# google-research/rigl

Measured on AMD Instinct MI355X. Metric: images/sec/node, ResNet-50 80% ERK RigL step, higher is better.
Workload: dtype bf16

## Files before the change

### include/rigl_hip.h

```cpp
#ifndef RIGL_HIP_H_
#define RIGL_HIP_H_

#include <stddef.h>
#include <stdint.h>

#ifdef __cplusplus
extern "C" {
#endif

#define RIGL_ABI_VERSION 2

typedef void* rigl_stream_t;
typedef uint16_t rigl_bf16;

enum {
  RIGL_OK = 0,
  RIGL_EINVAL = -1,
  RIGL_ELAUNCH = -2,
  RIGL_EWORKSPACE = -3,
  RIGL_EUNSUPPORTED = -4
};

int rigl_version(void);
uint32_t rigl_crc32c(const void* data, size_t n, uint32_t crc);
// ... 282 lines not shown
                      const float* gamma, const float* save_mean,
                      const float* save_invstd, const float* save_scale,
                      const float* save_shift, int32_t relu, rigl_bf16* dx,
                      rigl_bf16* dresidual , float* dgamma,
                      float* dbeta, const float* stats, int32_t stats_parts,
                      void* workspace, size_t workspace_bytes, rigl_stream_t stream);

int rigl_bn_add_bn_fwd(int64_t m, int32_t c, const rigl_bf16* x, const rigl_bf16* x2,
                       const float* scale2, const float* shift2,
                       const float* gamma, const float* beta, float* running_mean,
                       float* running_var, float momentum, float eps, int32_t relu,
                       rigl_bf16* y, float* save_mean, float* save_invstd,
                       float* save_scale, float* save_shift, const float* stats,
                       int32_t stats_parts, uint8_t* relu_bits ,
                       void* workspace, size_t workspace_bytes, rigl_stream_t stream);
size_t rigl_bn_add_bn_bwd_workspace_bytes(int64_t m, int32_t c);
int rigl_bn_add_bn_bwd(int64_t m, int32_t c, const rigl_bf16* x, const rigl_bf16* x2,
                       const uint8_t* relu_bits, const rigl_bf16* dy,
                       const float* gamma, const float* save_mean, const float* save_invstd,
                       const float* gamma2, const float* save_mean2, const float* save_invstd2,
                       rigl_bf16* dx, rigl_bf16* dx2, float* dgamma, float* dbeta,
                       float* dgamma2, float* dbeta2, void* workspace,
                       size_t workspace_bytes, rigl_stream_t stream);

int rigl_stateless_random(float* out, int64_t n, int32_t seed0, int32_t seed1,
                          int32_t dist, float scale, float shift,
                          rigl_stream_t stream);
typedef struct {
  float* out;
  int64_t n;
// ... 118 lines not shown
```

### rigl_amd/_lib.py

```python
import ctypes as C
import os

_HERE = os.path.dirname(os.path.abspath(__file__))
ABI_VERSION = 2
LIB_PATH = os.environ.get('RIGL_HIP_LIB') or os.path.join(_HERE, 'lib', 'librigl_hip.so')

RIGL_OK = 0
RIGL_EINVAL = -1
RIGL_ELAUNCH = -2
RIGL_EWORKSPACE = -3
RIGL_EUNSUPPORTED = -4
COUNTS_PER_LAYER = 8
MAGPRUNE_COUNTS_PER_LAYER = 4
PROF_KINDS = ('conv_fwd', 'conv_dgrad', 'conv_wgrad', 'prune_regrow',
              'sgd_momentum', 'pack_weights', 'conv_bwd', 'depthwise', 'masked_adam', 'magnitude_prune')

GROW_ZEROS, GROW_GRAD_SCALE, GROW_GRAD_SIGN, GROW_EXPLICIT = 0, 1, 2, 3
MOMRESET_ZEROS, MOMRESET_GRAD = 0, 1


class RiglError(RuntimeError):

  def __init__(self, code, msg):
    super().__init__('librigl_hip: error %d: %s' % (code, msg))
# ... 124 lines not shown
    'rigl_bn_fwd': (C.c_int, [_I64, _I32, _P, _P, _P, _P, _P, _P, _F, _F, _I32, _P, _P, _P, _P, _P, _P, _SZ, _P]),
    'rigl_bn_fwd_stats': (C.c_int, [_I64, _I32, _P, _P, _P, _P, _P, _P, _F, _F, _I32, _P, _P, _P, _P, _P, _P, _I32, _P, _P, _SZ, _P]),
    'rigl_bn_bwd': (C.c_int, [_I64, _I32, _P, _P, _P, _P, _P, _P, _P, _P, _P, _I32, _P, _P, _P, _P, _P, _SZ, _P]),
    'rigl_bn_bwd_stats': (C.c_int, [_I64, _I32, _P, _P, _P, _P, _P, _P, _P, _P, _P, _I32, _P, _P, _P, _P, _P, _I32, _P, _SZ, _P]),
    'rigl_bn_bwd_reduce': (C.c_int, [_I64, _I32, _P, _P, _P, _P, _P, _P, _I32, _P, _P, _P, _P, _SZ, _P]),
    'rigl_crc32c': (C.c_uint32, [_P, _SZ, C.c_uint32]),
    'rigl_stateless_random': (C.c_int, [_P, _I64, _I32, _I32, _I32, _F, _F, _P]),
    'rigl_stateless_random_batched': (C.c_int, [C.POINTER(RandomItem), _I32, _P]),
    'rigl_dropout_fwd': (C.c_int, [_P, _P, _P, _I64, _I32, _F, _I32, _P, _P]),
    'rigl_dropout_bwd': (C.c_int, [_P, _P, _P, _I64, _I32, _F, _P]),
    'rigl_dropout_advance': (C.c_int, [_P, _P]),
    'rigl_maxpool_fwd': (C.c_int, [C.POINTER(ConvDesc), _P, _P, _P, _P]),
    'rigl_maxpool_bwd': (C.c_int, [C.POINTER(ConvDesc), _P, _P, _P, _P]),
    'rigl_bn_fwd_statistics': (C.c_int, [_I64, _I32, _P, _P, _P, _P, _P, _F, _F, _P, _P, _P, _P, _P, _I32, _P, _SZ, _P]),
    'rigl_bn_add_bn_fwd': (C.c_int, [_I64, _I32, _P, _P, _P, _P, _P, _P, _P, _P, _F, _F, _I32, _P, _P, _P, _P, _P, _P, _I32, _P, _P, _SZ, _P]),
    'rigl_bn_add_bn_bwd_workspace_bytes': (_SZ, [_I64, _I32]),
    'rigl_bn_add_bn_bwd': (C.c_int, [_I64, _I32, _P, _P, _P, _P, _P, _P, _P, _P, _P, _P, _P, _P, _P, _P, _P, _P, _P, _SZ, _P]),
    'rigl_bn_relu_maxpool_fwd': (C.c_int, [C.POINTER(ConvDesc), _P, _P, _P, _P, _P, _P]),
    'rigl_bn_relu_maxpool_bwd_workspace_bytes': (_SZ, [C.POINTER(ConvDesc)]),
    'rigl_bn_relu_maxpool_bwd': (C.c_int, [C.POINTER(ConvDesc), _P, _P, _P, _P, _P, _P, _P, _P, _P, _P, _P, _P, _SZ, _P]),
    'rigl_global_avgpool_fwd': (C.c_int, [_I32, _I32, _I32, _P, _P, _P]),
    'rigl_global_avgpool_bwd': (C.c_int, [_I32, _I32, _I32, _P, _P, _P]),
    'rigl_softmax_xent': (C.c_int, [_I32, _I32, _P, _P, _F, _F, _P, _P, _P]),
    'rigl_global_avgpool_bwd_relu': (C.c_int, [_I32, _I32, _I32, _P, _P, _P, _P]),
    'rigl_conv2d_fwd_takes_relu_epilogue': (C.c_int32, [C.POINTER(ConvDesc)]),
    'rigl_conv2d_bwd_takes_relu_epilogue': (C.c_int32, [C.POINTER(ConvDesc)]),
    'rigl_masked_conv2d_fwd_relu': (C.c_int, [C.POINTER(ConvDesc), _P, _P, _P, _P, _SZ, _P]),
    'rigl_masked_conv2d_bwd_relu': (C.c_int, [C.POINTER(ConvDesc), _P, _P, _P, _P, _P, _P, _SZ, _P]),
    'rigl_relu_fwd': (C.c_int, [_I64, _P, _P, _P]),
    'rigl_relu_bwd': (C.c_int, [_I64, _P, _P, _P, _P]),
# ... 50 lines not shown
```

### rigl_amd/csrc/bn.hip

```cpp
#include "common.hpp"

namespace rigl {
namespace kbn {

constexpr int THREADS = 256;
constexpr int MAX_PARTS = 512;

__device__ __forceinline__ float bf_lo(uint32_t w) { return __uint_as_float(w << 16); }
__device__ __forceinline__ float bf_hi(uint32_t w) { return __uint_as_float(w & 0xFFFF0000u); }
__device__ __forceinline__ uint32_t f2bf(float f) {
  uint32_t u = __float_as_uint(f);
  if ((u & 0x7FFFFFFFu) > 0x7F800000u) return (u >> 16) | 0x40u;
  u += 0x7FFFu + ((u >> 16) & 1u);
  return u >> 16;
}
typedef __attribute__((ext_vector_type(2))) __bf16 bf16x2_t;
typedef __attribute__((ext_vector_type(2))) float f32x2_t;
__device__ __forceinline__ uint32_t pack2(float a, float b) {
  const f32x2_t v = {a, b};
  return __builtin_bit_cast(uint32_t, __builtin_convertvector(v, bf16x2_t));
}
__device__ __forceinline__ void unpack8(const uint4& v, float f[8]) {
  f[0] = bf_lo(v.x); f[1] = bf_hi(v.x); f[2] = bf_lo(v.y); f[3] = bf_hi(v.y);
  f[4] = bf_lo(v.z); f[5] = bf_hi(v.z); f[6] = bf_lo(v.w); f[7] = bf_hi(v.w);
// ... 99 lines not shown
      for (int j = 0; j < 16; ++j) own[j] += oth[j];
      if (s > 1) {
#pragma unroll
        for (int j = 0; j < 16; ++j) red[threadIdx.x][j] = own[j];
      }
    }
    if (s > 1) __syncthreads();
  }
  if (ty == 0 && c_ok) {
    float* p = partial + ((int64_t)blockIdx.x * 2) * G.C + cgi * 8;
#pragma unroll
    for (int j = 0; j < 8; ++j) { p[j] = own[j]; p[G.C + j] = own[8 + j]; }
  }
}

template <int CL>
__device__ __forceinline__ void sum_partials(const Geom& G, const float* __restrict__ partial, double& s0, double& s1,
                                             int& c, bool& leader) {
  constexpr int PL = THREADS / CL;
  __shared__ double acc[2][PL][CL + 1];
  const int cl = threadIdx.x % CL, pl = threadIdx.x / CL;
  c = blockIdx.x * CL + cl;
  double a0 = 0.0, a1 = 0.0;
  if (c < G.C) {
#ifndef RIGL_BN_FIN_FLIGHT
#define RIGL_BN_FIN_FLIGHT 16
#endif
    constexpr int FLIGHT = RIGL_BN_FIN_FLIGHT;
    for (int p0 = pl; p0 < G.parts; p0 += PL * FLIGHT) {
      float v0[FLIGHT], v1[FLIGHT];
#pragma unroll
      for (int j = 0; j < FLIGHT; ++j) {
        const int p = p0 + j * PL;
        const int pc = p < G.parts ? p : G.parts - 1;
        const float l0 = partial[((int64_t)pc * 2) * G.C + c], l1 = partial[((int64_t)pc * 2 + 1) * G.C + c];
        v0[j] = p < G.parts ? l0 : 0.f;
        v1[j] = p < G.parts ? l1 : 0.f;
      }
#pragma unroll
      for (int j = 0; j < FLIGHT; ++j) { a0 += (double)v0[j]; a1 += (double)v1[j]; }
    }
  }
  acc[0][pl][cl] = a0; acc[1][pl][cl] = a1;
  __syncthreads();
  leader = pl == 0 && c < G.C;
  s0 = s1 = 0.0;
  if constexpr (CL == 1) {
    __shared__ double acc2[2][16];
    if (threadIdx.x < 16) {
      double t0 = 0.0, t1 = 0.0;
#pragma unroll
      for (int k = 0; k < 16; ++k) { t0 += acc[0][threadIdx.x * 16 + k][0]; t1 += acc[1][threadIdx.x * 16 + k][0]; }
      acc2[0][threadIdx.x] = t0; acc2[1][threadIdx.x] = t1;
    }
    __syncthreads();
    if (leader) {
#pragma unroll
      for (int k = 0; k < 16; ++k) { s0 += acc2[0][k]; s1 += acc2[1][k]; }
    }
  } else if (leader) {
#pragma unroll 8
    for (int k = 0; k < PL; ++k) { s0 += acc[0][k][cl]; s1 += acc[1][k][cl]; }
  }
}

template <int CL>
__global__ __launch_bounds__(THREADS) void k_fwd_finalize(Geom G, const float* __restrict__ partial,
                                                           const uint16_t* __restrict__ x ,
                                                           const float* __restrict__ gamma, const float* __restrict__ beta,
                                                           float* __restrict__ running_mean, float* __restrict__ running_var,
                                                           float momentum, float eps, float* __restrict__ save_mean,
                                                           float* __restrict__ save_invstd, float* __restrict__ scale,
                                                           float* __restrict__ shift) {
  double s0, s1; int c; bool leader;
  sum_partials<CL>(G, partial, s0, s1, c, leader);
  if (!leader) return;
  const double m = (double)G.M;
  double k = 0.0;
  if (x) {
    const float a = __uint_as_float((uint32_t)x[c] << 16), b = __uint_as_float((uint32_t)x[(G.M / 2) * G.C + c] << 16),
                e = __uint_as_float((uint32_t)x[(G.M - 1) * G.C + c] << 16);
    k = (double)pivot3(a, b, e);
  }
  const double dm = s0 / m;
  const double mean = k + dm;
  double var = s1 / m - dm * dm;
  if (var < 0.0) var = 0.0;
  const float invstd = (float)(1.0 / sqrt(var + (double)eps));
  save_mean[c] = (float)mean;
  save_invstd[c] = invstd;
  const float sc = gamma[c] * invstd;
  scale[c] = sc;
  shift[c] = beta[c] - (float)mean * sc;
  if (running_mean) {
    const double unbiased = G.M > 1 ? var * m / (m - 1.0) : var;
    running_mean[c] = (1.f - momentum) * running_mean[c] + momentum * (float)mean;
    running_var[c] = (1.f - momentum) * running_var[c] + momentum * (float)unbiased;
  }
}

template <bool RELU, bool HAS_RES>
__global__ __launch_bounds__(THREADS) void k_fwd_apply(Geom G, const uint16_t* __restrict__ x, const uint16_t* __restrict__ res,
                                                        const float* __restrict__ scale, const float* __restrict__ shift,
                                                        uint16_t* __restrict__ y, uint8_t* __restrict__ mbits) {
  extern __shared__ __attribute__((aligned(16))) float prm[];
  const bool fixed = G.fixed != 0;
  float psc[8], psh[8];
  if (fixed) {
    const int c0 = (int)(((int64_t)blockIdx.x * THREADS + threadIdx.x) % G.cg) * 8;
    ld8f(scale + c0, psc); ld8f(shift + c0, psh);
  } else {
    for (int i = threadIdx.x; i < G.C; i += THREADS) { prm[i] = scale[i]; prm[G.C + i] = shift[i]; }
    __syncthreads();
// ... 16 lines not shown
      if (HAS_RES) v += rv[j];
      o[j] = RELU ? fmaxf(v, 0.f) : v;
    }
    uint4 out;
    out.x = pack2(o[0], o[1]); out.y = pack2(o[2], o[3]); out.z = pack2(o[4], o[5]); out.w = pack2(o[6], o[7]);
    st16(y + i * 8, out, G.nt);
    if (RELU && mbits) {
      uint32_t mb = 0u;
#pragma unroll
      for (int j = 0; j < 8; ++j) mb |= (o[j] > 0.f ? 1u : 0u) << j;
      mbits[i] = (uint8_t)mb;
    }
  }
}

template <int CL>
__global__ __launch_bounds__(THREADS) void k_bwd_finalize(Geom G, const float* __restrict__ partial,
                                                           const float* __restrict__ gamma, const float* __restrict__ invstd,
                                                           float* __restrict__ dgamma, float* __restrict__ dbeta,
                                                           float* __restrict__ coef ) {
  double s0, s1; int c; bool leader;
  sum_partials<CL>(G, partial, s0, s1, c, leader);
  if (!leader) return;
  dbeta[c] = (float)s0;
  dgamma[c] = (float)s1;
  coef[c] = gamma[c] * invstd[c];
  coef[G.C + c] = (float)(s0 / (double)G.M);
  coef[2 * G.C + c] = (float)(s1 / (double)G.M);
}

template <bool RELU, int MSK, bool HAS_DRES>
__global__ __launch_bounds__(THREADS) void k_bwd_apply(Geom G, const uint16_t* __restrict__ x, const uint16_t* __restrict__ y,
                                                        const uint8_t* __restrict__ mbits,
                                                        const uint16_t* __restrict__ dy, const float* __restrict__ mean,
                                                        const float* __restrict__ invstd, const float* __restrict__ scale,
                                                        const float* __restrict__ shift, const float* __restrict__ coef,
                                                        uint16_t* __restrict__ dx, uint16_t* __restrict__ dres) {
  extern __shared__ __attribute__((aligned(16))) float prm[];
  const bool fixed = G.fixed != 0;
  float pm[8], pis[8], pa[8], pb[8], pc[8], psc[8], psh[8];
  if (fixed) {
// ... 157 lines not shown
    if (s > 1) __syncthreads();
  }
  if (ty == 0 && c_ok) {
    float* p = partial + ((int64_t)blockIdx.x * 2) * G.C + cgi * 8;
    float* p2 = partial2 + ((int64_t)blockIdx.x * 2) * G.C + cgi * 8;
#pragma unroll
    for (int j = 0; j < 8; ++j) {
      p[j] = own[j]; p[G.C + j] = own[8 + j];
      p2[j] = own[j]; p2[G.C + j] = own[16 + j];
    }
  }
}

struct FinSet { const float* partial; const float* gamma; const float* invstd; float* dgamma; float* dbeta; float* coef; };

template <int CL>
__global__ __launch_bounds__(THREADS) void k_bwd_finalize_pair(Geom G, FinSet s0, FinSet s1) {
  const FinSet& f = blockIdx.y == 0 ? s0 : s1;
  double a0, a1; int c; bool leader;
  sum_partials<CL>(G, f.partial, a0, a1, c, leader);
  if (!leader) return;
  f.dbeta[c] = (float)a0;
  f.dgamma[c] = (float)a1;
  f.coef[c] = f.gamma[c] * f.invstd[c];
  f.coef[G.C + c] = (float)(a0 / (double)G.M);
  f.coef[2 * G.C + c] = (float)(a1 / (double)G.M);
}

__global__ __launch_bounds__(THREADS) void k_bwd_apply_pair(Geom G, const uint16_t* __restrict__ x, const uint16_t* __restrict__ x2,
                                                             const uint8_t* __restrict__ mbits, const uint16_t* __restrict__ dy,
                                                             const float* __restrict__ mean, const float* __restrict__ invstd,
                                                             const float* __restrict__ mean2, const float* __restrict__ invstd2,
                                                             const float* __restrict__ coef, const float* __restrict__ coef2,
                                                             uint16_t* __restrict__ dx, uint16_t* __restrict__ dx2) {
  extern __shared__ __attribute__((aligned(16))) float prm[];
  const bool fixed = G.fixed != 0;
  float q[10][8];
  if (fixed) {
    const int c0 = (int)(((int64_t)blockIdx.x * THREADS + threadIdx.x) % G.cg) * 8;
// ... 83 lines not shown

static unsigned apply_grid(Geom& g) {
#ifndef RIGL_BN_APPLY_PER_THREAD
#define RIGL_BN_APPLY_PER_THREAD 2
#endif
#ifndef RIGL_BN_APPLY_CAP
#define RIGL_BN_APPLY_CAP 16384
#endif
  int64_t b = (g.M * g.cg + THREADS * RIGL_BN_APPLY_PER_THREAD - 1) / (THREADS * RIGL_BN_APPLY_PER_THREAD);
  if (b > RIGL_BN_APPLY_CAP) b = RIGL_BN_APPLY_CAP;
  if (b < 1) b = 1;
  g.fixed = (RIGL_TUNE("bn_regs", 1) != 0 && (b * THREADS) % g.cg == 0) ? 1 : 0;
  return (unsigned)b;
}

void launch_bwd_finalize(int64_t m, int c, const float* partial, int parts, const float* gamma, const float* invstd,
                         float* dgamma, float* dbeta, float* coef, hipStream_t st) {
  Geom g = make_geom(m, c);
  g.parts = parts;
  if (parts > MAX_PARTS)
    hipLaunchKernelGGL(k_bwd_finalize<4>, dim3((unsigned)((c + 3) / 4)), dim3(THREADS), 0, st, g, partial, gamma, invstd,
                       dgamma, dbeta, coef);
  else
    hipLaunchKernelGGL(k_bwd_finalize<16>, dim3((unsigned)((c + 15) / 16)), dim3(THREADS), 0, st, g, partial, gamma, invstd,
                       dgamma, dbeta, coef);
}

static int fwd_statistics(Geom& g, int32_t c, const rigl_bf16* x, const float* gamma, const float* beta,
                          float* running_mean, float* running_var, float momentum, float eps, float* save_mean,
                          float* save_invstd, float* save_scale, float* save_shift, const float* stats,
                          int32_t stats_parts, void* workspace, size_t workspace_bytes, hipStream_t st) {
  const float* partial = stats;
  if (!stats) {
    const size_t need = rigl_bn_workspace_bytes(g.M, c);
    if (!workspace || workspace_bytes < need) return fail(RIGL_EWORKSPACE, "rigl_bn_fwd: workspace %zu < %zu", workspace_bytes, need);
    float* ws_partial = static_cast<float*>(workspace);
    dim3 rgrid((unsigned)g.parts, (unsigned)((g.cg + g.tpr - 1) / g.tpr));
    hipLaunchKernelGGL((k_reduce<0, false, 0>), rgrid, dim3(THREADS), 0, st, g, x, nullptr, nullptr, nullptr, nullptr, nullptr,
                       nullptr, nullptr, ws_partial);
    partial = ws_partial;
  } else {
    g.parts = stats_parts;
  }
  if (g.parts > 1024 && RIGL_TUNE("bn_fin1", 1) != 0)
    hipLaunchKernelGGL(k_fwd_finalize<1>, dim3((unsigned)c), dim3(THREADS), 0, st, g, partial, stats ? nullptr : reinterpret_cast<const uint16_t*>(x), gamma,
                       beta, running_mean, running_var, momentum, eps, save_mean, save_invstd, save_scale, save_shift);
  else if (g.parts > 256)
    hipLaunchKernelGGL(k_fwd_finalize<4>, dim3((unsigned)((c + 3) / 4)), dim3(THREADS), 0, st, g, partial, stats ? nullptr : reinterpret_cast<const uint16_t*>(x), gamma,
                       beta, running_mean, running_var, momentum, eps, save_mean, save_invstd, save_scale, save_shift);
  else
    hipLaunchKernelGGL(k_fwd_finalize<16>, dim3((unsigned)((c + 15) / 16)), dim3(THREADS), 0, st, g, partial, stats ? nullptr : reinterpret_cast<const uint16_t*>(x), gamma,
                       beta, running_mean, running_var, momentum, eps, save_mean, save_invstd, save_scale, save_shift);
  return RIGL_OK;
}

}
}

extern "C" {

size_t rigl_bn_workspace_bytes(int64_t m, int32_t c) {
  if (m <= 0 || c <= 0) return 0;
  rigl::kbn::Geom g = rigl::kbn::make_geom(m, c);
  return rigl::align_up((size_t)g.parts * 2 * c * 4, 256) + rigl::align_up((size_t)3 * c * 4, 256);
}

int rigl_bn_fwd_stats(int64_t m, int32_t c, const rigl_bf16* x, const rigl_bf16* residual, const float* gamma,
// ... 61 lines not shown
      !save_scale || !save_shift)
    return fail(RIGL_EINVAL, "rigl_bn_add_bn_fwd: bad arguments");
  if (c % 8) return fail(RIGL_EUNSUPPORTED, "rigl_bn_add_bn_fwd: channels %% 8 != 0");
  if (4 * (size_t)c * 4 > 65536) return fail(RIGL_EUNSUPPORTED, "rigl_bn_add_bn_fwd: too many channels for the LDS parameter cache");
  if (stats && stats_parts <= 0) return fail(RIGL_EINVAL, "rigl_bn_add_bn_fwd: stats_parts must be positive");
  hipStream_t st = as_stream(stream);
  Geom g = make_geom(m, c);
  int rc = fwd_statistics(g, c, x, gamma, beta, running_mean, running_var, momentum, eps, save_mean, save_invstd,
                          save_scale, save_shift, stats, stats_parts, workspace, workspace_bytes, st);
  if (rc) return rc;
  dim3 agrid(apply_grid(g));
  const size_t lds = g.fixed ? 0 : (size_t)4 * c * 4;
  if (relu) hipLaunchKernelGGL(k_fwd_apply_pair<true>, agrid, dim3(THREADS), lds, st, g, x, x2, save_scale, save_shift, scale2, shift2, y, relu_bits);
  else hipLaunchKernelGGL(k_fwd_apply_pair<false>, agrid, dim3(THREADS), lds, st, g, x, x2, save_scale, save_shift, scale2, shift2, y, nullptr);
  RIGL_CHECK_LAUNCH("rigl_bn_add_bn_fwd");
  return RIGL_OK;
}

size_t rigl_bn_add_bn_bwd_workspace_bytes(int64_t m, int32_t c) { return 2 * rigl_bn_workspace_bytes(m, c); }

int rigl_bn_add_bn_bwd(int64_t m, int32_t c, const rigl_bf16* x, const rigl_bf16* x2, const uint8_t* relu_bits,
                       const rigl_bf16* dy, const float* gamma, const float* save_mean, const float* save_invstd,
                       const float* gamma2, const float* save_mean2, const float* save_invstd2, rigl_bf16* dx,
                       rigl_bf16* dx2, float* dgamma, float* dbeta, float* dgamma2, float* dbeta2, void* workspace,
                       size_t workspace_bytes, rigl_stream_t stream) {
  using namespace rigl;
  using namespace rigl::kbn;
  if (m <= 0 || c <= 0 || !x || !x2 || !relu_bits || !dy || !gamma || !save_mean || !save_invstd || !gamma2 || !save_mean2 ||
      !save_invstd2 || !dx || !dx2 || !dgamma || !dbeta || !dgamma2 || !dbeta2)
    return fail(RIGL_EINVAL, "rigl_bn_add_bn_bwd: bad arguments");
// ... 7 lines not shown
  if (lds > 65536 && !big_lds) return fail(RIGL_ELAUNCH, "rigl_bn_add_bn_bwd: cannot raise the dynamic LDS limit");
  hipStream_t st = as_stream(stream);
  Geom g = make_geom(m, c);
  const size_t half = rigl_bn_workspace_bytes(m, c);
  const size_t part_bytes = align_up((size_t)g.parts * 2 * c * 4, 256);
  char* w0 = static_cast<char*>(workspace);
  float* partial = reinterpret_cast<float*>(w0);
  float* coef = reinterpret_cast<float*>(w0 + part_bytes);
  float* partial2 = reinterpret_cast<float*>(w0 + half);
  float* coef2 = reinterpret_cast<float*>(w0 + half + part_bytes);
  dim3 rgrid((unsigned)g.parts, (unsigned)((g.cg + g.tpr - 1) / g.tpr));
  hipLaunchKernelGGL(k_reduce_pair, rgrid, dim3(THREADS), 0, st, g, x, x2, relu_bits, dy, save_mean, save_invstd, save_mean2,
                     save_invstd2, partial, partial2);
  const FinSet f0 = {partial, gamma, save_invstd, dgamma, dbeta, coef};
  const FinSet f1 = {partial2, gamma2, save_invstd2, dgamma2, dbeta2, coef2};
  hipLaunchKernelGGL(k_bwd_finalize_pair<16>, dim3((unsigned)((c + 15) / 16), 2), dim3(THREADS), 0, st, g, f0, f1);
  const dim3 pgrid(apply_grid(g));
  hipLaunchKernelGGL(k_bwd_apply_pair, pgrid, dim3(THREADS), g.fixed ? 0 : lds, st, g, x, x2, relu_bits, dy, save_mean, save_invstd,
                     save_mean2, save_invstd2, coef, coef2, dx, dx2);
  RIGL_CHECK_LAUNCH("rigl_bn_add_bn_bwd");
  return RIGL_OK;
}

static int bn_bwd_impl(int64_t m, int32_t c, const rigl_bf16* x, const rigl_bf16* y, const uint8_t* relu_bits,
                       const rigl_bf16* dy, const float* gamma,
                       const float* save_mean, const float* save_invstd, const float* save_scale, const float* save_shift,
                       int32_t relu, rigl_bf16* dx, rigl_bf16* dresidual, float* dgamma, float* dbeta,
                       const float* stats, int32_t stats_parts, float* coef_out, void* workspace,
                       size_t workspace_bytes, rigl_stream_t stream) {
  using namespace rigl;
  using namespace rigl::kbn;
// ... 12 lines not shown
  float* coef = coef_out ? coef_out : reinterpret_cast<float*>(static_cast<char*>(workspace) + align_up((size_t)g.parts * 2 * c * 4, 256));
  dim3 rgrid((unsigned)g.parts, (unsigned)((g.cg + g.tpr - 1) / g.tpr));
  const int msk = relu_bits ? 2 : (y ? 1 : 0);
  const float* red = partial;
  if (stats) {
    red = stats;
    g.parts = stats_parts;
  } else {
#define RIGL_BWD_REDUCE(R, K) hipLaunchKernelGGL((k_reduce<1, R, K>), rgrid, dim3(THREADS), 0, st, g, x, y, relu_bits, dy, save_mean, save_invstd, save_scale, save_shift, partial)
    if (!relu) RIGL_BWD_REDUCE(false, 0);
    else if (msk == 2) RIGL_BWD_REDUCE(true, 2);
    else if (msk == 1) RIGL_BWD_REDUCE(true, 1);
    else RIGL_BWD_REDUCE(true, 0);
#undef RIGL_BWD_REDUCE
  }
  if (g.parts > MAX_PARTS)
    hipLaunchKernelGGL(k_bwd_finalize<4>, dim3((unsigned)((c + 3) / 4)), dim3(THREADS), 0, st, g, red, gamma,
                       save_invstd, dgamma, dbeta, coef);
  else
    hipLaunchKernelGGL(k_bwd_finalize<16>, dim3((unsigned)((c + 15) / 16)), dim3(THREADS), 0, st, g, red, gamma,
                       save_invstd, dgamma, dbeta, coef);
  if (coef_out) {
    RIGL_CHECK_LAUNCH("rigl_bn_bwd_reduce");
    return RIGL_OK;
  }
  dim3 agrid(apply_grid(g));
  const size_t lds = g.fixed ? 0 : (size_t)7 * c * 4;
#define RIGL_BWD_APPLY(R, K, D) hipLaunchKernelGGL((k_bwd_apply<R, K, D>), agrid, dim3(THREADS), lds, st, g, x, y, relu_bits, dy, save_mean, save_invstd, save_scale, save_shift, coef, dx, dresidual)
  const bool dres = dresidual != nullptr;
  if (!relu) { if (dres) RIGL_BWD_APPLY(false, 0, true); else RIGL_BWD_APPLY(false, 0, false); }
  else if (msk == 2) { if (dres) RIGL_BWD_APPLY(true, 2, true); else RIGL_BWD_APPLY(true, 2, false); }
  else if (msk == 1) { if (dres) RIGL_BWD_APPLY(true, 1, true); else RIGL_BWD_APPLY(true, 1, false); }
  else { if (dres) RIGL_BWD_APPLY(true, 0, true); else RIGL_BWD_APPLY(true, 0, false); }
#undef RIGL_BWD_APPLY
  RIGL_CHECK_LAUNCH("rigl_bn_bwd");
  return RIGL_OK;
// ... 98 lines not shown
```

### rigl_amd/ops.py

```python
import ctypes as C
import os

import torch

from rigl_amd import _lib
from rigl_amd._lib import (ConvDesc, PackLayer, PruneRegrowLayer,
                           PruneRegrowParams, RiglError, check)

_workspaces = {}


_raw_stream = getattr(torch._C, '_cuda_getCurrentRawStream', None)
_cur_device = getattr(torch._C, '_cuda_getDevice', None)


def _stream():
  if _raw_stream is not None and _cur_device is not None:
    return C.c_void_p(_raw_stream(_cur_device()))
  return C.c_void_p(torch.cuda.current_stream().cuda_stream)


def _ptr(t):
  return C.c_void_p(t.data_ptr()) if t is not None else C.c_void_p(0)

# ... 891 lines not shown
  _req(x2, torch.bfloat16, 'x2')
  if x2.shape != x.shape:
    raise ValueError('x2 must have the shape of x')
  m, c, ws, parts = _bn_plan(x, partials)
  y = torch.empty_like(x)
  saved = torch.empty((4, c), dtype=torch.float32, device=x.device)
  bits = torch.empty(x.numel() // 8, dtype=torch.uint8, device=x.device) if relu else None
  check(_lib.load().rigl_bn_add_bn_fwd(
      m, c, _ptr(x), _ptr(x2), _ptr(saved2[2]), _ptr(saved2[3]), _ptr(gamma), _ptr(beta), _ptr(running_mean),
      _ptr(running_var), float(momentum), float(eps), int(bool(relu)), _ptr(y), _ptr(saved[0]), _ptr(saved[1]),
      _ptr(saved[2]), _ptr(saved[3]), _ptr(partials), parts, _ptr(bits),
      _ptr(ws), ws.numel() if ws is not None else 0, _stream()))
  return y, saved, bits


def bn_add_bn_bwd(x, x2, relu_bits, dy, gamma, saved, gamma2, saved2, dgamma, dbeta, dgamma2, dbeta2):
  _req(x, torch.bfloat16, 'x')
  _req(x2, torch.bfloat16, 'x2')
  _req(dy, torch.bfloat16, 'dy')
  _req(relu_bits, torch.uint8, 'relu_bits')
  c = x.shape[-1]
  m = x.numel() // c
  lib = _lib.load()
  ws = workspace(lib.rigl_bn_add_bn_bwd_workspace_bytes(m, c), x.device)
  dx, dx2 = torch.empty_like(x), torch.empty_like(x2)
  check(lib.rigl_bn_add_bn_bwd(m, c, _ptr(x), _ptr(x2), _ptr(relu_bits), _ptr(dy), _ptr(gamma), _ptr(saved[0]), _ptr(saved[1]),
                               _ptr(gamma2), _ptr(saved2[0]), _ptr(saved2[1]), _ptr(dx), _ptr(dx2), _ptr(dgamma), _ptr(dbeta),
                               _ptr(dgamma2), _ptr(dbeta2), _ptr(ws), ws.numel(), _stream()))
  return dx, dx2

# ... 198 lines not shown
```

### rigl_amd/workloads/nn.py

```python
import os

import torch
import torch.nn.functional as F

from rigl_amd import variables as V
from rigl_amd.pruning_layers import bias_tensor, stats_outputs

BATCH_NORM_DECAY = 0.9
BATCH_NORM_EPSILON = 1e-5
_DW_STATS = os.environ.get('RIGL_DW_STATS', '1') != '0'


def activation_dtype(precision=None):
  if precision is None:
    from rigl_amd import ops
    precision = 'float32' if ops.tune_get('k1_fp32', 0) == 1 else 'bfloat16'
  if precision not in ('bfloat16', 'float32'):
    raise ValueError('precision must be bfloat16 or float32, got %r' % (precision,))
  return torch.float32 if precision == 'float32' else torch.bfloat16


def nchw_view(x):
  return x.permute(0, 3, 1, 2)

# ... 78 lines not shown
      ctx.addend_holder.fill(dy, bits)
      return dx, dy, None, None, None, None, None, None, None
    dx, dres = ops.bn_bwd(x, None, dy, bn.gamma.data, saved, ctx.relu,
                          bn.gamma.grad, bn.beta.grad,
                          want_dres=ctx.has_res and ctx.needs_input_grad[1],
                          relu_bits=bits, partials=part)
    return dx, dres, None, None, None, None, None, None, None


class _BnAddBnFn(torch.autograd.Function):

  @staticmethod
  def forward(ctx, x, x2, bn, bn2, partials, partials2):
    from rigl_amd import ops
    x, x2 = x.contiguous(), x2.contiguous()
    saved2 = ops.bn_statistics(x2, bn2.gamma.data, bn2.beta.data, bn2.moving_mean, bn2.moving_variance,
                               1.0 - bn2.decay, bn2.eps, partials=partials2)
    y, saved, bits = ops.bn_add_bn_fwd(x, x2, saved2, bn.gamma.data, bn.beta.data, bn.moving_mean, bn.moving_variance,
                                       1.0 - bn.decay, bn.eps, True, partials=partials)
    ctx.bn, ctx.bn2 = bn, bn2
    ctx.save_for_backward(x, x2, saved, saved2, bits)
    return y

  @staticmethod
  def backward(ctx, dy):
    from rigl_amd import ops
    x, x2, saved, saved2, bits = ctx.saved_tensors
    bn, bn2 = ctx.bn, ctx.bn2
    dx, dx2 = ops.bn_add_bn_bwd(x, x2, bits, dy.contiguous(), bn.gamma.data, saved, bn2.gamma.data, saved2,
                                bn.gamma.grad, bn.beta.grad, bn2.gamma.grad, bn2.beta.grad)
    return dx, dx2, None, None, None, None


_BN_PAIR_FUSED = os.environ.get('RIGL_BN_PAIR', '1') != '0'
# ... 352 lines not shown
```

Before: 12820.

## Fuse paired BN forward finalize into one launch and prefetch per-channel params

Adds a rigl_bn_add_bn_fwd_pair entry point. It finalizes the statistics of both batch norms feeding a residual add in a single two-row grid launch, then runs the paired apply, replacing separate statistics and add-BN calls and cutting kernel launches and host round trips per bottleneck block. Finalize kernels gain a BATCH variant that loads gamma, beta, running stats and pivot samples before the partial-sum reduction, so that latency overlaps with the reduction. The reduction also uses a deeper in-flight load count when the part count is large. The extra template variants add register pressure, and the fused path only runs when both producers supply partial sums.

```diff
diff --git a/include/rigl_hip.h b/include/rigl_hip.h
--- a/include/rigl_hip.h
+++ b/include/rigl_hip.h
@@ -320,6 +320,17 @@
                        float* save_scale, float* save_shift, const float* stats,
                        int32_t stats_parts, uint8_t* relu_bits ,
                        void* workspace, size_t workspace_bytes, rigl_stream_t stream);
+int rigl_bn_add_bn_fwd_pair(int64_t m, int32_t c, const rigl_bf16* x, const rigl_bf16* x2,
+                            const float* gamma, const float* beta,
+                            float* running_mean , float* running_var,
+                            float momentum, float eps, const float* gamma2, const float* beta2,
+                            float* running_mean2 , float* running_var2,
+                            float momentum2, float eps2, int32_t relu, rigl_bf16* y,
+                            float* save_mean, float* save_invstd, float* save_scale,
+                            float* save_shift, float* save_mean2, float* save_invstd2,
+                            float* save_scale2, float* save_shift2, const float* stats,
+                            int32_t stats_parts, const float* stats2, int32_t stats_parts2,
+                            uint8_t* relu_bits , rigl_stream_t stream);
 size_t rigl_bn_add_bn_bwd_workspace_bytes(int64_t m, int32_t c);
 int rigl_bn_add_bn_bwd(int64_t m, int32_t c, const rigl_bf16* x, const rigl_bf16* x2,
                        const uint8_t* relu_bits, const rigl_bf16* dy,
diff --git a/rigl_amd/_lib.py b/rigl_amd/_lib.py
--- a/rigl_amd/_lib.py
+++ b/rigl_amd/_lib.py
@@ -162,6 +162,8 @@
     'rigl_maxpool_bwd': (C.c_int, [C.POINTER(ConvDesc), _P, _P, _P, _P]),
     'rigl_bn_fwd_statistics': (C.c_int, [_I64, _I32, _P, _P, _P, _P, _P, _F, _F, _P, _P, _P, _P, _P, _I32, _P, _SZ, _P]),
     'rigl_bn_add_bn_fwd': (C.c_int, [_I64, _I32, _P, _P, _P, _P, _P, _P, _P, _P, _F, _F, _I32, _P, _P, _P, _P, _P, _P, _I32, _P, _P, _SZ, _P]),
+    'rigl_bn_add_bn_fwd_pair': (C.c_int, [_I64, _I32, _P, _P, _P, _P, _P, _P, _F, _F, _P, _P, _P, _P, _F, _F, _I32, _P,
+                                          _P, _P, _P, _P, _P, _P, _P, _P, _P, _I32, _P, _I32, _P, _P]),
     'rigl_bn_add_bn_bwd_workspace_bytes': (_SZ, [_I64, _I32]),
     'rigl_bn_add_bn_bwd': (C.c_int, [_I64, _I32, _P, _P, _P, _P, _P, _P, _P, _P, _P, _P, _P, _P, _P, _P, _P, _P, _P, _SZ, _P]),
     'rigl_bn_relu_maxpool_fwd': (C.c_int, [C.POINTER(ConvDesc), _P, _P, _P, _P, _P, _P]),
diff --git a/rigl_amd/csrc/bn.hip b/rigl_amd/csrc/bn.hip
--- a/rigl_amd/csrc/bn.hip
+++ b/rigl_amd/csrc/bn.hip
@@ -137,7 +137,28 @@
   }
 }
 
-template <int CL>
+#ifndef RIGL_BN_FIN_FLIGHT
+#define RIGL_BN_FIN_FLIGHT 16
+#endif
+template <int FLIGHT>
+__device__ __forceinline__ void sum_lane(const Geom& G, const float* __restrict__ partial, int c, int pl, int PL, double& a0,
+                                         double& a1) {
+  for (int p0 = pl; p0 < G.parts; p0 += PL * FLIGHT) {
+    float v0[FLIGHT], v1[FLIGHT];
+#pragma unroll
+    for (int j = 0; j < FLIGHT; ++j) {
+      const int p = p0 + j * PL;
+      const int pc = p < G.parts ? p : G.parts - 1;
+      const float l0 = partial[((int64_t)pc * 2) * G.C + c], l1 = partial[((int64_t)pc * 2 + 1) * G.C + c];
+      v0[j] = p < G.parts ? l0 : 0.f;
+      v1[j] = p < G.parts ? l1 : 0.f;
+    }
+#pragma unroll
+    for (int j = 0; j < FLIGHT; ++j) { a0 += (double)v0[j]; a1 += (double)v1[j]; }
+  }
+}
+
+template <int CL, int BATCH>
 __device__ __forceinline__ void sum_partials(const Geom& G, const float* __restrict__ partial, double& s0, double& s1,
                                              int& c, bool& leader) {
   constexpr int PL = THREADS / CL;
@@ -146,23 +167,8 @@
   c = blockIdx.x * CL + cl;
   double a0 = 0.0, a1 = 0.0;
   if (c < G.C) {
-#ifndef RIGL_BN_FIN_FLIGHT
-#define RIGL_BN_FIN_FLIGHT 16
-#endif
-    constexpr int FLIGHT = RIGL_BN_FIN_FLIGHT;
-    for (int p0 = pl; p0 < G.parts; p0 += PL * FLIGHT) {
-      float v0[FLIGHT], v1[FLIGHT];
-#pragma unroll
-      for (int j = 0; j < FLIGHT; ++j) {
-        const int p = p0 + j * PL;
-        const int pc = p < G.parts ? p : G.parts - 1;
-        const float l0 = partial[((int64_t)pc * 2) * G.C + c], l1 = partial[((int64_t)pc * 2 + 1) * G.C + c];
-        v0[j] = p < G.parts ? l0 : 0.f;
-        v1[j] = p < G.parts ? l1 : 0.f;
-      }
-#pragma unroll
-      for (int j = 0; j < FLIGHT; ++j) { a0 += (double)v0[j]; a1 += (double)v1[j]; }
-    }
+    if (BATCH && CL == 16 && G.parts > PL * RIGL_BN_FIN_FLIGHT) sum_lane<2 * RIGL_BN_FIN_FLIGHT>(G, partial, c, pl, PL, a0, a1);
+    else sum_lane<RIGL_BN_FIN_FLIGHT>(G, partial, c, pl, PL, a0, a1);
   }
   acc[0][pl][cl] = a0; acc[1][pl][cl] = a1;
   __syncthreads();
@@ -187,7 +193,62 @@
   }
 }
 
+struct FwdPrm { float gamma, beta, rmean, rvar, xa, xb, xe; };
+__device__ __forceinline__ FwdPrm fwd_prm(const Geom& G, int c, const uint16_t* __restrict__ x, const float* __restrict__ gamma,
+                                          const float* __restrict__ beta, const float* __restrict__ running_mean,
+                                          const float* __restrict__ running_var) {
+  FwdPrm q;
+  q.gamma = gamma[c]; q.beta = beta[c];
+  q.rmean = q.rvar = 0.f;
+  if (running_mean) { q.rmean = running_mean[c]; q.rvar = running_var[c]; }
+  q.xa = q.xb = q.xe = 0.f;
+  if (x) {
+    q.xa = __uint_as_float((uint32_t)x[c] << 16); q.xb = __uint_as_float((uint32_t)x[(G.M / 2) * G.C + c] << 16);
+    q.xe = __uint_as_float((uint32_t)x[(G.M - 1) * G.C + c] << 16);
+  }
+  return q;
+}
+
+template <int BATCH>
+__device__ __forceinline__ void fwd_finish(const Geom& G, int c, double s0, double s1, const FwdPrm& q, const uint16_t* __restrict__ x,
+                                           const float* __restrict__ gamma, const float* __restrict__ beta,
+                                           float* __restrict__ running_mean, float* __restrict__ running_var, float momentum,
+                                           float eps, float* __restrict__ save_mean, float* __restrict__ save_invstd,
+                                           float* __restrict__ scale, float* __restrict__ shift) {
+  const double m = (double)G.M;
+  double k = 0.0;
+  if (x) {
+    if (BATCH) k = (double)pivot3(q.xa, q.xb, q.xe);
+    else {
+      const float a = __uint_as_float((uint32_t)x[c] << 16), b = __uint_as_float((uint32_t)x[(G.M / 2) * G.C + c] << 16),
+                  e = __uint_as_float((uint32_t)x[(G.M - 1) * G.C + c] << 16);
+      k = (double)pivot3(a, b, e);
+    }
+  }
+  const double dm = s0 / m;
+  const double mean = k + dm;
+  double var = s1 / m - dm * dm;
+  if (var < 0.0) var = 0.0;
+  const float invstd = (float)(1.0 / sqrt(var + (double)eps));
+  save_mean[c] = (float)mean;
+  save_invstd[c] = invstd;
+  const float sc = (BATCH ? q.gamma : gamma[c]) * invstd;
+  scale[c] = sc;
+  shift[c] = (BATCH ? q.beta : beta[c]) - (float)mean * sc;
+  if (running_mean) {
+    const double unbiased = G.M > 1 ? var * m / (m - 1.0) : var;
+    running_mean[c] = (1.f - momentum) * (BATCH ? q.rmean : running_mean[c]) + momentum * (float)mean;
+    running_var[c] = (1.f - momentum) * (BATCH ? q.rvar : running_var[c]) + momentum * (float)unbiased;
+  }
+}
+
 template <int CL>
+__device__ __forceinline__ int fin_channel(const Geom& G) {
+  const int c = blockIdx.x * CL + threadIdx.x % CL;
+  return c < G.C ? c : G.C - 1;
+}
+
+template <int CL, int BATCH>
 __global__ __launch_bounds__(THREADS) void k_fwd_finalize(Geom G, const float* __restrict__ partial,
                                                            const uint16_t* __restrict__ x ,
                                                            const float* __restrict__ gamma, const float* __restrict__ beta,
@@ -195,31 +256,28 @@
                                                            float momentum, float eps, float* __restrict__ save_mean,
                                                            float* __restrict__ save_invstd, float* __restrict__ scale,
                                                            float* __restrict__ shift) {
+  FwdPrm q = {};
+  if (BATCH) q = fwd_prm(G, fin_channel<CL>(G), x, gamma, beta, running_mean, running_var);
   double s0, s1; int c; bool leader;
-  sum_partials<CL>(G, partial, s0, s1, c, leader);
+  sum_partials<CL, BATCH>(G, partial, s0, s1, c, leader);
   if (!leader) return;
-  const double m = (double)G.M;
-  double k = 0.0;
-  if (x) {
-    const float a = __uint_as_float((uint32_t)x[c] << 16), b = __uint_as_float((uint32_t)x[(G.M / 2) * G.C + c] << 16),
-                e = __uint_as_float((uint32_t)x[(G.M - 1) * G.C + c] << 16);
-    k = (double)pivot3(a, b, e);
-  }
-  const double dm = s0 / m;
-  const double mean = k + dm;
-  double var = s1 / m - dm * dm;
-  if (var < 0.0) var = 0.0;
-  const float invstd = (float)(1.0 / sqrt(var + (double)eps));
-  save_mean[c] = (float)mean;
-  save_invstd[c] = invstd;
-  const float sc = gamma[c] * invstd;
-  scale[c] = sc;
-  shift[c] = beta[c] - (float)mean * sc;
-  if (running_mean) {
-    const double unbiased = G.M > 1 ? var * m / (m - 1.0) : var;
-    running_mean[c] = (1.f - momentum) * running_mean[c] + momentum * (float)mean;
-    running_var[c] = (1.f - momentum) * running_var[c] + momentum * (float)unbiased;
-  }
+  fwd_finish<BATCH>(G, c, s0, s1, q, x, gamma, beta, running_mean, running_var, momentum, eps, save_mean, save_invstd, scale, shift);
+}
+
+struct FwdSet {
+  const float* partial; const float* gamma; const float* beta; float* running_mean; float* running_var;
+  float* save_mean; float* save_invstd; float* scale; float* shift; float momentum, eps; int parts;
+};
+template <int CL>
+__global__ __launch_bounds__(THREADS) void k_fwd_finalize_pair(Geom G, FwdSet f0, FwdSet f1) {
+  const FwdSet& f = blockIdx.y == 0 ? f0 : f1;
+  G.parts = f.parts;
+  const FwdPrm q = fwd_prm(G, fin_channel<CL>(G), nullptr, f.gamma, f.beta, f.running_mean, f.running_var);
+  double s0, s1; int c; bool leader;
+  sum_partials<CL, 1>(G, f.partial, s0, s1, c, leader);
+  if (!leader) return;
+  fwd_finish<1>(G, c, s0, s1, q, nullptr, f.gamma, f.beta, f.running_mean, f.running_var, f.momentum, f.eps, f.save_mean, f.save_invstd,
+                f.scale, f.shift);
 }
 
 template <bool RELU, bool HAS_RES>
@@ -266,17 +324,20 @@
   }
 }
 
-template <int CL>
+template <int CL, int BATCH>
 __global__ __launch_bounds__(THREADS) void k_bwd_finalize(Geom G, const float* __restrict__ partial,
                                                            const float* __restrict__ gamma, const float* __restrict__ invstd,
                                                            float* __restrict__ dgamma, float* __restrict__ dbeta,
                                                            float* __restrict__ coef ) {
+  float ga = 0.f, is = 0.f;
+  if (BATCH) { const int cc = fin_channel<CL>(G); ga = gamma[cc]; is = invstd[cc]; }
   double s0, s1; int c; bool leader;
-  sum_partials<CL>(G, partial, s0, s1, c, leader);
+  sum_partials<CL, BATCH>(G, partial, s0, s1, c, leader);
   if (!leader) return;
+  if (!BATCH) { ga = gamma[c]; is = invstd[c]; }
   dbeta[c] = (float)s0;
   dgamma[c] = (float)s1;
-  coef[c] = gamma[c] * invstd[c];
+  coef[c] = ga * is;
   coef[G.C + c] = (float)(s0 / (double)G.M);
   coef[2 * G.C + c] = (float)(s1 / (double)G.M);
 }
@@ -464,15 +525,17 @@
 
 struct FinSet { const float* partial; const float* gamma; const float* invstd; float* dgamma; float* dbeta; float* coef; };
 
-template <int CL>
+template <int CL, int BATCH>
 __global__ __launch_bounds__(THREADS) void k_bwd_finalize_pair(Geom G, FinSet s0, FinSet s1) {
   const FinSet& f = blockIdx.y == 0 ? s0 : s1;
+  float ga = 0.f, is = 0.f;
+  if (BATCH) { const int cc = fin_channel<CL>(G); ga = f.gamma[cc]; is = f.invstd[cc]; }
   double a0, a1; int c; bool leader;
-  sum_partials<CL>(G, f.partial, a0, a1, c, leader);
+  sum_partials<CL, BATCH>(G, f.partial, a0, a1, c, leader);
   if (!leader) return;
   f.dbeta[c] = (float)a0;
   f.dgamma[c] = (float)a1;
-  f.coef[c] = f.gamma[c] * f.invstd[c];
+  f.coef[c] = BATCH ? ga * is : f.gamma[c] * f.invstd[c];
   f.coef[G.C + c] = (float)(a0 / (double)G.M);
   f.coef[2 * G.C + c] = (float)(a1 / (double)G.M);
 }
@@ -586,16 +649,33 @@
   return (unsigned)b;
 }
 
+static bool fin_batch() { return RIGL_TUNE("bn_fin_batch", 1) != 0; }
+
+static void bwd_finalize(const Geom& g, int c, const float* partial, const float* gamma, const float* invstd, float* dgamma,
+                         float* dbeta, float* coef, hipStream_t st) {
+#define RIGL_BWD_FIN(CL, B) hipLaunchKernelGGL((k_bwd_finalize<CL, B>), dim3((unsigned)((c + CL - 1) / CL)), dim3(THREADS), 0, st, g, partial, gamma, invstd, dgamma, dbeta, coef)
+  if (g.parts > MAX_PARTS) { if (fin_batch()) RIGL_BWD_FIN(4, 1); else RIGL_BWD_FIN(4, 0); }
+  else { if (fin_batch()) RIGL_BWD_FIN(16, 1); else RIGL_BWD_FIN(16, 0); }
+#undef RIGL_BWD_FIN
+}
+
 void launch_bwd_finalize(int64_t m, int c, const float* partial, int parts, const float* gamma, const float* invstd,
                          float* dgamma, float* dbeta, float* coef, hipStream_t st) {
   Geom g = make_geom(m, c);
   g.parts = parts;
-  if (parts > MAX_PARTS)
-    hipLaunchKernelGGL(k_bwd_finalize<4>, dim3((unsigned)((c + 3) / 4)), dim3(THREADS), 0, st, g, partial, gamma, invstd,
-                       dgamma, dbeta, coef);
-  else
-    hipLaunchKernelGGL(k_bwd_finalize<16>, dim3((unsigned)((c + 15) / 16)), dim3(THREADS), 0, st, g, partial, gamma, invstd,
-                       dgamma, dbeta, coef);
+  bwd_finalize(g, c, partial, gamma, invstd, dgamma, dbeta, coef, st);
+}
+
+static int fwd_finalize_cl(int parts) { return parts > 1024 && RIGL_TUNE("bn_fin1", 1) != 0 ? 1 : (parts > 256 ? 4 : 16); }
+static void fwd_finalize(const Geom& g, int c, const float* partial, const uint16_t* x, const float* gamma, const float* beta,
+                         float* running_mean, float* running_var, float momentum, float eps, float* save_mean,
+                         float* save_invstd, float* save_scale, float* save_shift, hipStream_t st) {
+#define RIGL_FWD_FIN(CL, B) hipLaunchKernelGGL((k_fwd_finalize<CL, B>), dim3((unsigned)((c + CL - 1) / CL)), dim3(THREADS), 0, st, g, partial, x, gamma, beta, running_mean, running_var, momentum, eps, save_mean, save_invstd, save_scale, save_shift)
+  const int cl = fwd_finalize_cl(g.parts);
+  if (cl == 1) RIGL_FWD_FIN(1, 0);
+  else if (cl == 4) { if (fin_batch()) RIGL_FWD_FIN(4, 1); else RIGL_FWD_FIN(4, 0); }
+  else { if (fin_batch()) RIGL_FWD_FIN(16, 1); else RIGL_FWD_FIN(16, 0); }
+#undef RIGL_FWD_FIN
 }
 
 static int fwd_statistics(Geom& g, int32_t c, const rigl_bf16* x, const float* gamma, const float* beta,
@@ -614,15 +694,8 @@
   } else {
     g.parts = stats_parts;
   }
-  if (g.parts > 1024 && RIGL_TUNE("bn_fin1", 1) != 0)
-    hipLaunchKernelGGL(k_fwd_finalize<1>, dim3((unsigned)c), dim3(THREADS), 0, st, g, partial, stats ? nullptr : reinterpret_cast<const uint16_t*>(x), gamma,
-                       beta, running_mean, running_var, momentum, eps, save_mean, save_invstd, save_scale, save_shift);
-  else if (g.parts > 256)
-    hipLaunchKernelGGL(k_fwd_finalize<4>, dim3((unsigned)((c + 3) / 4)), dim3(THREADS), 0, st, g, partial, stats ? nullptr : reinterpret_cast<const uint16_t*>(x), gamma,
-                       beta, running_mean, running_var, momentum, eps, save_mean, save_invstd, save_scale, save_shift);
-  else
-    hipLaunchKernelGGL(k_fwd_finalize<16>, dim3((unsigned)((c + 15) / 16)), dim3(THREADS), 0, st, g, partial, stats ? nullptr : reinterpret_cast<const uint16_t*>(x), gamma,
-                       beta, running_mean, running_var, momentum, eps, save_mean, save_invstd, save_scale, save_shift);
+  fwd_finalize(g, c, partial, stats ? nullptr : reinterpret_cast<const uint16_t*>(x), gamma, beta, running_mean, running_var,
+               momentum, eps, save_mean, save_invstd, save_scale, save_shift, st);
   return RIGL_OK;
 }
 
@@ -714,6 +787,47 @@
   if (relu) hipLaunchKernelGGL(k_fwd_apply_pair<true>, agrid, dim3(THREADS), lds, st, g, x, x2, save_scale, save_shift, scale2, shift2, y, relu_bits);
   else hipLaunchKernelGGL(k_fwd_apply_pair<false>, agrid, dim3(THREADS), lds, st, g, x, x2, save_scale, save_shift, scale2, shift2, y, nullptr);
   RIGL_CHECK_LAUNCH("rigl_bn_add_bn_fwd");
+  return RIGL_OK;
+}
+
+int rigl_bn_add_bn_fwd_pair(int64_t m, int32_t c, const rigl_bf16* x, const rigl_bf16* x2, const float* gamma,
+                            const float* beta, float* running_mean, float* running_var, float momentum, float eps,
+                            const float* gamma2, const float* beta2, float* running_mean2, float* running_var2,
+                            float momentum2, float eps2, int32_t relu, rigl_bf16* y, float* save_mean, float* save_invstd,
+                            float* save_scale, float* save_shift, float* save_mean2, float* save_invstd2, float* save_scale2,
+                            float* save_shift2, const float* stats, int32_t stats_parts, const float* stats2,
+                            int32_t stats_parts2, uint8_t* relu_bits, rigl_stream_t stream) {
+  using namespace rigl;
+  using namespace rigl::kbn;
+  if (m <= 0 || c <= 0 || !x || !x2 || !gamma || !beta || !gamma2 || !beta2 || !y || !save_mean || !save_invstd || !save_scale ||
+      !save_shift || !save_mean2 || !save_invstd2 || !save_scale2 || !save_shift2 || !stats || !stats2 ||
+      (!running_mean) != (!running_var) || (!running_mean2) != (!running_var2))
+    return fail(RIGL_EINVAL, "rigl_bn_add_bn_fwd_pair: bad arguments");
+  if (c % 8) return fail(RIGL_EUNSUPPORTED, "rigl_bn_add_bn_fwd_pair: channels %% 8 != 0");
+  if (4 * (size_t)c * 4 > 65536) return fail(RIGL_EUNSUPPORTED, "rigl_bn_add_bn_fwd_pair: too many channels for the LDS parameter cache");
+  if (stats_parts <= 0 || stats_parts2 <= 0) return fail(RIGL_EINVAL, "rigl_bn_add_bn_fwd_pair: stats_parts must be positive");
+  hipStream_t st = as_stream(stream);
+  Geom g = make_geom(m, c);
+  const int cl = fwd_finalize_cl(stats_parts);
+  if (fin_batch() && cl != 1 && cl == fwd_finalize_cl(stats_parts2)) {
+    const FwdSet f0 = {stats, gamma, beta, running_mean, running_var, save_mean, save_invstd, save_scale, save_shift, momentum, eps, stats_parts};
+    const FwdSet f1 = {stats2, gamma2, beta2, running_mean2, running_var2, save_mean2, save_invstd2, save_scale2, save_shift2, momentum2, eps2, stats_parts2};
+#define RIGL_FWD_FIN_PAIR(CL) hipLaunchKernelGGL(k_fwd_finalize_pair<CL>, dim3((unsigned)((c + CL - 1) / CL), 2), dim3(THREADS), 0, st, g, f0, f1)
+    if (cl == 4) RIGL_FWD_FIN_PAIR(4); else RIGL_FWD_FIN_PAIR(16);
+#undef RIGL_FWD_FIN_PAIR
+  } else {
+    g.parts = stats_parts2;
+    fwd_finalize(g, c, stats2, nullptr, gamma2, beta2, running_mean2, running_var2, momentum2, eps2, save_mean2, save_invstd2,
+                 save_scale2, save_shift2, st);
+    g.parts = stats_parts;
+    fwd_finalize(g, c, stats, nullptr, gamma, beta, running_mean, running_var, momentum, eps, save_mean, save_invstd, save_scale,
+                 save_shift, st);
+  }
+  dim3 agrid(apply_grid(g));
+  const size_t lds = g.fixed ? 0 : (size_t)4 * c * 4;
+  if (relu) hipLaunchKernelGGL(k_fwd_apply_pair<true>, agrid, dim3(THREADS), lds, st, g, x, x2, save_scale, save_shift, save_scale2, save_shift2, y, relu_bits);
+  else hipLaunchKernelGGL(k_fwd_apply_pair<false>, agrid, dim3(THREADS), lds, st, g, x, x2, save_scale, save_shift, save_scale2, save_shift2, y, nullptr);
+  RIGL_CHECK_LAUNCH("rigl_bn_add_bn_fwd_pair");
   return RIGL_OK;
 }
 
@@ -751,7 +865,8 @@
                      save_invstd2, partial, partial2);
   const FinSet f0 = {partial, gamma, save_invstd, dgamma, dbeta, coef};
   const FinSet f1 = {partial2, gamma2, save_invstd2, dgamma2, dbeta2, coef2};
-  hipLaunchKernelGGL(k_bwd_finalize_pair<16>, dim3((unsigned)((c + 15) / 16), 2), dim3(THREADS), 0, st, g, f0, f1);
+  if (fin_batch()) hipLaunchKernelGGL((k_bwd_finalize_pair<16, 1>), dim3((unsigned)((c + 15) / 16), 2), dim3(THREADS), 0, st, g, f0, f1);
+  else hipLaunchKernelGGL((k_bwd_finalize_pair<16, 0>), dim3((unsigned)((c + 15) / 16), 2), dim3(THREADS), 0, st, g, f0, f1);
   const dim3 pgrid(apply_grid(g));
   hipLaunchKernelGGL(k_bwd_apply_pair, pgrid, dim3(THREADS), g.fixed ? 0 : lds, st, g, x, x2, relu_bits, dy, save_mean, save_invstd,
                      save_mean2, save_invstd2, coef, coef2, dx, dx2);
@@ -794,12 +909,7 @@
     else RIGL_BWD_REDUCE(true, 0);
 #undef RIGL_BWD_REDUCE
   }
-  if (g.parts > MAX_PARTS)
-    hipLaunchKernelGGL(k_bwd_finalize<4>, dim3((unsigned)((c + 3) / 4)), dim3(THREADS), 0, st, g, red, gamma,
-                       save_invstd, dgamma, dbeta, coef);
-  else
-    hipLaunchKernelGGL(k_bwd_finalize<16>, dim3((unsigned)((c + 15) / 16)), dim3(THREADS), 0, st, g, red, gamma,
-                       save_invstd, dgamma, dbeta, coef);
+  bwd_finalize(g, c, red, gamma, save_invstd, dgamma, dbeta, coef, st);
   if (coef_out) {
     RIGL_CHECK_LAUNCH("rigl_bn_bwd_reduce");
     return RIGL_OK;
diff --git a/rigl_amd/ops.py b/rigl_amd/ops.py
--- a/rigl_amd/ops.py
+++ b/rigl_amd/ops.py
@@ -929,6 +929,27 @@
   return y, saved, bits
 
 
+def bn_add_bn_fwd_pair(x, x2, gamma, beta, running_mean, running_var, momentum, eps, gamma2, beta2, running_mean2, running_var2,
+                       momentum2, eps2, relu, partials, partials2):
+  _req(x2, torch.bfloat16, 'x2')
+  if x2.shape != x.shape:
+    raise ValueError('x2 must have the shape of x')
+  if partials is None or partials2 is None:
+    raise ValueError('bn_add_bn_fwd_pair needs the partial sums of both producers')
+  m, c, _, parts = _bn_plan(x, partials)
+  _, _, _, parts2 = _bn_plan(x2, partials2)
+  y = torch.empty_like(x)
+  saved = torch.empty((4, c), dtype=torch.float32, device=x.device)
+  saved2 = torch.empty((4, c), dtype=torch.float32, device=x.device)
+  bits = torch.empty(x.numel() // 8, dtype=torch.uint8, device=x.device) if relu else None
+  check(_lib.load().rigl_bn_add_bn_fwd_pair(
+      m, c, _ptr(x), _ptr(x2), _ptr(gamma), _ptr(beta), _ptr(running_mean), _ptr(running_var), float(momentum), float(eps),
+      _ptr(gamma2), _ptr(beta2), _ptr(running_mean2), _ptr(running_var2), float(momentum2), float(eps2), int(bool(relu)),
+      _ptr(y), _ptr(saved[0]), _ptr(saved[1]), _ptr(saved[2]), _ptr(saved[3]), _ptr(saved2[0]), _ptr(saved2[1]),
+      _ptr(saved2[2]), _ptr(saved2[3]), _ptr(partials), parts, _ptr(partials2), parts2, _ptr(bits), _stream()))
+  return y, saved, saved2, bits
+
+
 def bn_add_bn_bwd(x, x2, relu_bits, dy, gamma, saved, gamma2, saved2, dgamma, dbeta, dgamma2, dbeta2):
   _req(x, torch.bfloat16, 'x')
   _req(x2, torch.bfloat16, 'x2')
diff --git a/rigl_amd/workloads/nn.py b/rigl_amd/workloads/nn.py
--- a/rigl_amd/workloads/nn.py
+++ b/rigl_amd/workloads/nn.py
@@ -116,10 +116,16 @@
   def forward(ctx, x, x2, bn, bn2, partials, partials2):
     from rigl_amd import ops
     x, x2 = x.contiguous(), x2.contiguous()
-    saved2 = ops.bn_statistics(x2, bn2.gamma.data, bn2.beta.data, bn2.moving_mean, bn2.moving_variance,
-                               1.0 - bn2.decay, bn2.eps, partials=partials2)
-    y, saved, bits = ops.bn_add_bn_fwd(x, x2, saved2, bn.gamma.data, bn.beta.data, bn.moving_mean, bn.moving_variance,
-                                       1.0 - bn.decay, bn.eps, True, partials=partials)
+    if partials is not None and partials2 is not None:
+      y, saved, saved2, bits = ops.bn_add_bn_fwd_pair(
+          x, x2, bn.gamma.data, bn.beta.data, bn.moving_mean, bn.moving_variance, 1.0 - bn.decay, bn.eps,
+          bn2.gamma.data, bn2.beta.data, bn2.moving_mean, bn2.moving_variance, 1.0 - bn2.decay, bn2.eps, True,
+          partials, partials2)
+    else:
+      saved2 = ops.bn_statistics(x2, bn2.gamma.data, bn2.beta.data, bn2.moving_mean, bn2.moving_variance,
+                                 1.0 - bn2.decay, bn2.eps, partials=partials2)
+      y, saved, bits = ops.bn_add_bn_fwd(x, x2, saved2, bn.gamma.data, bn.beta.data, bn.moving_mean, bn.moving_variance,
+                                         1.0 - bn.decay, bn.eps, True, partials=partials)
     ctx.bn, ctx.bn2 = bn, bn2
     ctx.save_for_backward(x, x2, saved, saved2, bits)
     return y
```

Result: no change. 12790 (-0.2%).
